# jkomijani/normflow_

Measured on AMD Instinct MI355X. Metric: lattice configs/sec (forward+logdet), higher is better.
Workload: dtype f32; 1 GPU; 32x32x32x32 phi^4 lattice, 8 RQ-spline coupling layers (knots_len 16, ConvAct 1-8-8-46, k=3, tanh), batch 1024 per GPU, forward + log|det J|, no_grad; global_batch=1024, parallelism=dp1

## Files before the change

include/normflow_hip.h:

```cpp
#ifndef NORMFLOW_HIP_H
#define NORMFLOW_HIP_H

#include <stddef.h>
#include <stdint.h>

#ifdef __cplusplus
extern "C" {
#endif

#define NF_VERSION 301

enum nf_dtype { NF_F32 = 0, NF_F64 = 1, NF_F16 = 2, NF_F16_FIELD = 3 };
enum nf_layout { NF_LAYOUT_FULL = 0, NF_LAYOUT_PAIR = 1 };
enum nf_extrap { NF_EXTRAP_NONE = 0, NF_EXTRAP_LINEAR = 1, NF_EXTRAP_ANTI = 2 };
enum nf_status {
  NF_OK = 0,
  NF_EINVAL = -1,
  NF_EWORKSPACE = -2,
  NF_ELAUNCH = -3
};

typedef struct nf_rqs_opts {
  int32_t m;
  int32_t extrap_left;
// ... 106 lines not shown

enum nf_pade_kind { NF_TANH = 1, NF_PADE11 = 11, NF_PADE22 = 22, NF_PADE32 = 32 };
size_t nf_pade_workspace_bytes(int64_t B, int64_t outer, int64_t C, int64_t inner);
int nf_pade(const void *x, const void *d0, const void *d1, const void *log0, void *y, void *logj, int64_t B,
            int64_t outer, int64_t C, int64_t inner, int kind, int inverse, int per_site, void *workspace,
            size_t workspace_bytes, int dtype, void *stream);
int nf_pade_vjp(const void *x, const void *d0, const void *d1, const void *grad_y, const void *grad_logj,
                void *grad_x, double *grad_d, int64_t B, int64_t outer, int64_t C, int64_t inner, int kind,
                int inverse, int per_site, void *workspace, size_t workspace_bytes, int dtype, void *stream);

int nf_spectral_supported(const int32_t *lat, int ndim, int dtype, int for_vjp);
size_t nf_spectral_workspace_bytes(const int32_t *lat, int ndim, int64_t B, int dtype);
int nf_spectral_filter(const void *x, const void *w_half, const void *zero_new, void *y, void *zero_old,
                       const int32_t *lat, int ndim, int64_t B, int dtype, void *stream);
int nf_spectral_filter_vjp(const void *x, const void *g, const void *w_half, int zero_replaced, void *gx, void *gw_half,
                           void *gzero, void *workspace, size_t workspace_bytes, const int32_t *lat, int ndim, int64_t B,
                           int dtype, void *stream);

int nf_conv_two_site(int cout, int compact, int l3, int k3);
int nf_conv_cin_pad(int cin);
int nf_conv_ntiles(int cout);
int nf_conv_packed_steps(int cin, int ntaps);
enum { NF_OUT_SPLIT16 = 2 };
int nf_conv_fwd(const void *in, const void *wfrag, const void *bias, void *out, int64_t B,
                const int32_t *lattice, const int32_t *ksize, int cin, int cout, int act,
                int compact, int active_parity, int dtype, void *stream);
enum { NF_WLAYOUT_FRAGMENT = 0, NF_WLAYOUT_ROWPACK = 1, NF_WLAYOUT_SPLIT16 = 2 };
int nf_conv_weight_layout(const int32_t *lattice, const int32_t *ksize, int cin, int cout, int compact,
                          int fused, int dtype);
int nf_conv_split16_supported(const int32_t *lattice, const int32_t *ksize, int cin, int cout, int act);
int nf_conv_affine_split16(const void *in16, const void *wsplit, const void *bias, const void *x_active, const void *log0,
                           void *y, void *logj, int64_t B, const int32_t *lattice, int active_parity, int inverse,
                           int flags, void *workspace, size_t workspace_bytes, void *stream);
int nf_conv_first_split16_supported(const int32_t *lattice, const int32_t *ksize, int cout, int act);
int nf_conv_first_split16(const void *in, const void *wsplit, const void *bias, void *out16, int64_t B,
                          const int32_t *lattice, int act, void *stream);
int nf_conv_fwd_split16(const void *in16, const void *wsplit, const void *bias, void *out16, int64_t B,
                        const int32_t *lattice, int act, void *stream);
typedef struct nf_conv_layer_plan {
  int32_t path;
  int32_t weight_layout;
  int32_t mt;
  int32_t two_site;
  int32_t packed;
  int32_t box[4];
  int32_t nbox[4];
  int32_t plane_stride;
  int32_t channels_per_pass;
  int32_t launches;
  int64_t lds_bytes;
  int64_t partials;
} nf_conv_layer_plan;
int nf_conv_plan(const int32_t *lattice, const int32_t *ksize, int cin, int cout, int compact, int fused, int dtype,
                 int64_t B, nf_conv_layer_plan *out);
int nf_conv_last_path(void);

enum { NF_CONV_UNIT_INPUT = 1, NF_CONV_SPLIT16_INPUT = 2, NF_CONV_FIELD_F16 = 4 };
int nf_conv_rqs_supported(int cout, int m);
int nf_conv_rqs_split16_supported(const int32_t *lattice, int cout, int m);
int nf_conv_rqs(const void *in, const void *wfrag, const void *bias, const void *x_active,
                const void *log0, void *y, void *logj, int64_t B, const int32_t *lattice,
                const int32_t *ksize, int cin, int cout, int active_parity,
                const nf_rqs_opts *opts, int inverse, int flags, void *workspace, size_t workspace_bytes,
                int dtype, void *stream);

int nf_phi4_action(const void *cfgs, void *action, int64_t B, const int32_t *lattice, double w0, double w2,
// ... 325 lines not shown
```

normflow__amd/_hip.py:

```python
import ctypes as C
import math
import os
import threading
import weakref

import torch

_HERE = os.path.dirname(os.path.abspath(__file__))
LIB_PATH = os.path.join(_HERE, "lib", "libnormflow_hip.so")

NF_F32, NF_F64, NF_F16, NF_F16_FIELD = 0, 1, 2, 3
LAYOUT_FULL, LAYOUT_PAIR = 0, 1
EXTRAP = {None: 0, 'none': 0, 'linear': 1, 'anti': 2, 'anti-periodic': 2}


OPT_SPLIT16, OPT_PIPE = 0, 1


class NormflowHipError(RuntimeError):
    pass


class RqsOpts(C.Structure):
    _fields_ = [("m", C.c_int32), ("extrap_left", C.c_int32), ("extrap_right", C.c_int32),
# ... 828 lines not shown
    lo = (w2 - hi.float()).half()
    out = torch.empty(27, 2, 64, 8, dtype=torch.float16, device=w.device)
    for k, part in enumerate((hi, lo)):
        out[:, k] = part.permute(2, 3, 0, 1).reshape(27, 64, 8)
    return out.contiguous()


def pack_conv_weight_split16_stacked(w):
    assert tuple(w.shape) == (8, 8, 3, 3, 3, 3)
    wr = w.reshape(8, 8, 9, 3, 3).float() * SPLIT16_WEIGHT_SCALE
    hi = wr.half()
    lo = (wr - hi.float()).half()
    parts = torch.stack((hi, lo))[:, :, :, :8]
    v = parts.reshape(2, 8, 8, 2, 4, 3, 3).permute(3, 5, 6, 4, 0, 1, 2)
    stacked = v.reshape(18, 64, 8)
    return torch.cat((stacked, pack_conv_weight_split16_two_site(w).reshape(54, 64, 8))).contiguous()


def pack_conv_weight_split16_first(w):
    assert tuple(w.shape) == (8, 1, 3, 3, 3, 3)
    wr = w.reshape(8, 27, 3).float() * SPLIT16_WEIGHT_SCALE
    w2 = wr.new_zeros(16, 32, 4)
    w2[:8, :27, :3] = wr
    w2[8:, :27, 1:] = wr
    hi = w2.half()
    lo = (w2 - hi.float()).half()
    out = torch.empty(4, 2, 64, 8, dtype=torch.float16, device=w.device)
    for k, part in enumerate((hi, lo)):
        v = part.reshape(16, 4, 4, 2, 4).permute(1, 2, 0, 3, 4)
        out[:, k] = v.reshape(4, 64, 8)
    return out.contiguous()


def conv_first_split16(x, weight, bias, act, weight_src=None):
    lib = load()
    B = x.shape[0]
    lat4 = _lat4(x.shape[2:])
    V = _sites(x.shape[2:])
    wsp = _cached_pack(weight if weight_src is None else weight_src, 'first16', pack_conv_weight_split16_first)
    bias = None if bias is None else bias.detach().float().contiguous()
    out = torch.empty((B, V, 16), dtype=torch.float16, device=x.device)
    for b0, b1 in _slabs(B, max(1, min(MAX_B, ((1 << 31) - 1) // V))):
        _check(lib.nf_conv_first_split16(_ptr(x[b0:b1]), _ptr(wsp), _ptr(bias), _ptr(out[b0:b1]), b1 - b0, lat4,
                                         int(act), _stream()), "nf_conv_first_split16")
    return out


def _split16_site_index(L3, device):
    slot = torch.arange(L3 // 2, device=device)
    return torch.stack((2 * slot, (2 * slot - 1) % L3))


def to_split16(h):
    B, Cc = h.shape[:2]
    L3 = h.shape[-1]
    if Cc != 8 or L3 % 2:
        raise NormflowHipError("to_split16: 8 channels and an even fastest axis expected")
    hp = h.reshape(B, 8, -1, L3).float()
    idx = _split16_site_index(L3, h.device)
    g = hp[..., idx].permute(0, 2, 3, 4, 1)
    hi = g.half()
    lo = (g - hi.float()).half()
    return torch.stack((hi, lo), dim=2).reshape(B, -1, 16).contiguous()


def from_split16(h16, lattice):
    B = h16.shape[0]
    L3 = lattice[-1]
    t = h16.reshape(B, -1, 2, 2, L3 // 2, 8).float()
    v = t[:, :, 0] + t[:, :, 1]
    idx = _split16_site_index(L3, h16.device)
    out = torch.empty((B, v.shape[1], L3, 8), dtype=torch.float32, device=h16.device)
# ... 96 lines not shown
        packed = build(probe)
        idx = (packed.reshape(-1).round().to(torch.int64) - 1).to(torch.int32).contiguous()
        ent = (idx, tuple(packed.shape))
        _GATHER_MAPS[key] = ent
    return ent


def _pack_by_gather(weight, gather_map):
    idx, shape = gather_map
    w = weight.contiguous()
    out = torch.empty(shape, dtype=w.dtype, device=w.device)
    _check(load().nf_gather_pad(_ptr(w), _ptr(idx), _ptr(out), idx.numel(), w.numel(), w.element_size(), _stream()), "nf_gather_pad")
    return out


def _conv_weight_map(shape, device, lat4, k4, cin, cout, compact, two_site, transposed, dtype_code):
    layout = load().nf_conv_weight_layout(lat4, k4, cin, cout, int(compact), 0, dtype_code)
    ksize = list(shape[2:])

    def build(w):
        if transposed:
            w = w.flip(list(range(2, w.dim()))).transpose(0, 1)
        if two_site:
            w2 = w.new_zeros((16, cin) + tuple(ksize[:-1]) + (ksize[-1] + 1,))
            w2[:cout, ..., :ksize[-1]] = w
            w2[8:8 + cout, ..., 1:] = w
            w = w2
        return conv_weight_for_layer(w, lat4, k4, cin, cout, compact, False, dtype_code)

    return _gather_map(shape, device, build, (transposed, two_site, tuple(lat4), tuple(k4), cin, cout, int(compact), dtype_code,
                                              layout))


def _conv_launch(x, weight, bias, act, compact, parity, weight_src=None, transposed=False):
    lib = load()
    B, cin = x.shape[:2]
    lat = list(x.shape[2:])
    cout, ksize = weight.shape[1 if transposed else 0], list(weight.shape[2:])
    d = len(lat)
    lat4, k4 = _lat4(lat, ksize)
    split16 = compact == 2
    if (split16 and cin == 1 and cout == 8 and d == 4 and x.dtype == torch.float32
            and _weights_fit_fp16(weight if weight_src is None else weight_src)
            and lib.nf_conv_first_split16_supported(lat4, k4, cout, act)):
        return conv_first_split16(x, weight, bias, act, weight_src)
    if split16 and not (lib.nf_conv_two_site(cout, 0, lat[-1], ksize[-1]) and cout == 8 and x.dtype == torch.float32):
        raise NormflowHipError("split-fp16 output needs an fp32 two-site layer with 8 output channels")
    two_site = bool(lib.nf_conv_two_site(cout, 0 if split16 else int(compact), lat[-1], ksize[-1]))
    eff_compact = False if (two_site and split16) else compact
    wfrag = _pack_by_gather(weight, _conv_weight_map(weight.shape, weight.device, lat4, k4, cin, cout, eff_compact, two_site,
                                                     transposed, _dtype_code(x)))
    V = _sites(lat)
    if split16:
        out = torch.empty((B, V, 16), dtype=torch.float16, device=x.device)
    else:
        out = torch.empty((B, cout, V // 2) if compact else (B, cout) + tuple(lat), dtype=x.dtype, device=x.device)
    for b0, b1 in _slabs(B):
        _check(lib.nf_conv_fwd(_ptr(x[b0:b1]), _ptr(wfrag), _ptr(bias), _ptr(out[b0:b1]), b1 - b0, lat4, k4,
                               cin, cout, act, int(compact), int(parity), _dtype_code(x), _stream()), "nf_conv_fwd")
    return out


def _compact_to_full(t, lattice, parity):
    _require_device(t)
    B, Cc, Vh = t.shape
    t = t.contiguous()
    full = torch.empty((B, Cc) + tuple(lattice), dtype=t.dtype, device=t.device)
    _check(load().nf_expand_pairs(_ptr(t), _ptr(full), B * Cc, _lat4(lattice), int(parity), _dtype_code(t), _stream()),
           "nf_expand_pairs")
    return full


def absmax_bits(t):
    bits = torch.empty(1, dtype=torch.int32, device=t.device)
    _check(load().nf_absmax_bits(_ptr(t), t.numel(), _ptr(bits), _stream()), "nf_absmax_bits")
    return bits


# ... 273 lines not shown
        lattice = tuple(h.shape[2:])
        lat4 = _lat4(lattice)
        cout = weight.shape[0]
        bits = absmax_bits(h)
        src, is16 = FusedLastRqsFn._source(h, bits, lat4)
        wsp = pack_conv_weight_split16(weight.detach().float())
        b = None if bias is None else bias.detach().float().contiguous()
        gz = torch.empty((B, cout, V // 2), dtype=torch.float32, device=h.device)
        gx = torch.empty_like(xpt)
        gy, glogj = gy.contiguous(), glogj.contiguous()
        work = torch.empty(4, dtype=torch.float32, device=h.device)
        _check(lib.nf_cotangent_pow2(_ptr(gy), gy.numel(), _ptr(glogj), glogj.numel(), _ptr(work), _stream()), "nf_cotangent_pow2")
        gys, gls = torch._foreach_mul([gy, glogj], work[2])
        _check(lib.nf_conv_rqs_split16_vjp(_ptr(src), is16, _ptr(wsp), _ptr(b), cout, _ptr(xpt), _ptr(gys),
                                           _ptr(gls), _ptr(gz), _ptr(gx), B, lat4, int(ctx.parity), _ptr(bits),
                                           C.byref(ctx.opts), int(bool(ctx.inverse)), _stream()), "nf_conv_rqs_split16_vjp")
        gh = gw = gb = None
        gbits = absmax_bits(gz)
        if ctx.needs_input_grad[0]:
            wt = weight.detach().flip([2, 3, 4, 5]).transpose(0, 1).contiguous()
            gh = conv_input_grad_split16(gz, wt, gbits, ctx.parity, lattice, weight)
        if ctx.needs_input_grad[1] or (bias is not None and ctx.needs_input_grad[2]):
            got = conv_weight_grad(h, gz, weight.shape[2:], gbits, ctx.parity)
            if got is not None:
                gw, gb = got
        if (ctx.needs_input_grad[0] and gh is None) or ((ctx.needs_input_grad[1] or ctx.needs_input_grad[2]) and gw is None):
            raise NormflowHipError("FusedLastRqsFn.backward: the split-fp16 gradient kernels refused a layer the forward pass took")
        if bias is None:
            gb = None
        torch._foreach_mul_([t for t in (gh, gw, gb, gx) if t is not None], work[3])
        return gh, gw, gb, gx, (glogj if ctx.has_log0 else None), None, None, None


def conv_layer(x, weight, bias, act=0, compact=False, parity=0):
    if torch.is_grad_enabled() and (x.requires_grad or weight.requires_grad or (bias is not None and bias.requires_grad)):
        if act == 5:
            return torch.abs(ConvFn.apply(x, weight, bias, 0, compact, parity))
        return ConvFn.apply(x, weight, bias, act, compact, parity)
    x = x.contiguous()
    return _conv_launch(x, weight.detach(), None if bias is None else bias.detach(), act, compact, parity, weight_src=weight)


def conv_affine_split16(h16, weight, bias, x_active, log0, parity, inverse, lattice, out=None):
    _require_device(h16, weight, bias, x_active, log0)
    lib = load()
    B, V = x_active.shape
    x_active = x_active.contiguous()
    lat4 = _lat4(lattice)
    def pack_affine(w):
        w8 = w.new_zeros((8, 8, 3, 3, 3, 3), dtype=torch.float32)
        w8[:2] = w.float()
        return pack_conv_weight_split16_stacked(w8)
    wsp = _cached_pack(weight, 'affine16s', pack_affine)
    b8 = torch.zeros(8, dtype=torch.float32, device=x_active.device)
    if bias is not None:
        b8[:2] = bias.detach().float()
    field16 = x_active.dtype == torch.float16
    if out is None:
        y = torch.empty_like(x_active)
        logj = torch.empty(B, dtype=torch.float32, device=x_active.device)
    else:
        y, logj = out
    ws = _workspace(min(B, MAX_B), V, x_active.device)
    for b0, b1 in _slabs(B):
        _check(lib.nf_conv_affine_split16(_ptr(h16[b0:b1]), _ptr(wsp), _ptr(b8), _ptr(x_active[b0:b1]), _ptr(_slab(log0, b0, b1)),
                                          _ptr(y[b0:b1]), _ptr(logj[b0:b1]), b1 - b0, lat4, int(parity), int(inverse),
                                          4 if field16 else 0, _ptr(ws), ws.numel(), _stream()), "nf_conv_affine_split16")
    return y, logj


def conv_rqs(h, weight, bias, x_active, log0, parity, opts, inverse, unit_input=False, lattice=None, out=None):
    _require_device(h, weight, bias, x_active, log0)
    lib = load()
# ... 1174 lines not shown
```

normflow__amd/csrc/nf_conv_c.hip:

```cpp
#include <hip/hip_runtime.h>
#include <hip/hip_fp16.h>
#include "nf_conv_core.h"

namespace nf {

typedef _Float16 f16x8 __attribute__((ext_vector_type(8)));
typedef _Float16 f16x4 __attribute__((ext_vector_type(4)));

namespace c2 {
constexpr int SEG = 32;
#ifndef NF_C2_IROW
#define NF_C2_IROW 80
#endif
constexpr int IROW = NF_C2_IROW;
constexpr int MAXROWS = 36;
constexpr int PLANE = 2 * MAXROWS * IROW;
constexpr int NPL = 4;
constexpr int LDS_BYTES = NPL * PLANE;
constexpr float kInvWScale = 1.0f / 1024.0f;
}

__device__ __forceinline__ float act_affine_c(float a, float c1, float c0, float al, float ga) {
  const float t = __builtin_amdgcn_exp2f(__builtin_fmaf(a, c1, c0));
  return __builtin_fmaf(al, __builtin_amdgcn_rcpf(1.0f + t), ga);
// ... 204 lines not shown
      stage_advance();
      stage_live = sci < ncols_my;
      if (stage_live) stage_issue(spl);
    }
    if (compute) {
#pragma unroll
      for (int t = 0; t < (HK ? 1 : 2); ++t) {
        if (tz[t] < NT) {
          f16x4 hi, lo;
#pragma unroll
          for (int r = 0; r < 4; ++r) {
            const float a = am[t][r] + ac[t][r];
            const float v = act_affine_c(a, kc1, kc0[r], kal, kga);
            const _Float16 h0 = static_cast<_Float16>(v);
            hi[r] = h0;
            lo[r] = static_cast<_Float16>(v - static_cast<float>(h0));
          }
          if (lane_ok) {
            unsigned char *d = (HK ? ((p & 8) ? ocol[1] : ocol[0]) : ocol[t]) + unsigned(z) * unsigned(RB) + lane_o;
            *reinterpret_cast<f16x4 *>(d) = hi;
            *reinterpret_cast<f16x4 *>(d + HB) = lo;
          }
        }
      }
    }
    lds_barrier();
    if (++pl > L2) {
      pl = -1;
      if (++cci < ncols_my) open_column(cci);
    }
  }
}

}

using namespace nf;

extern "C" int nf_conv_first_split16_supported(const int32_t *lattice, const int32_t *ksize, int cout, int act) {
  if (!nf::option(NF_OPT_SPLIT16) || !lattice || !ksize || cout != 8) return 0;
  if (act != kActTanh && act != kActSigmoid) return 0;
  for (int mu = 0; mu < 4; ++mu)
    if (ksize[mu] != 3) return 0;
  return split16_lattice_ok(lattice) ? 1 : 0;
}

extern "C" int nf_conv_first_split16(const void *in, const void *wsplit, const void *bias, void *out16, int64_t B,
                                     const int32_t *lattice, int act, void *stream_) {
  hipStream_t stream = static_cast<hipStream_t>(stream_);
  NF_REQUIRE(in && wsplit && out16 && lattice, "nf_conv_first_split16: NULL pointer");
  const int32_t k3[4] = {3, 3, 3, 3};
  NF_REQUIRE(nf_conv_first_split16_supported(lattice, k3, 8, act), "nf_conv_first_split16: layer not supported (needs a fastest axis of 32 + 16 n sites, even other extents, tanh / sigmoid)");
  NF_REQUIRE(B >= 0 && B <= 65535, "nf_conv_first_split16: batch outside [0, 65535]");
  if (B == 0) return NF_OK;
  ConvArgs A{};
  A.in = in; A.wfrag = wsplit; A.bias = bias; A.out = out16;
  set_lattice_k3(A, lattice);
  A.cin = 1; A.cout = 8; A.act = act;
  A.box[0] = lattice[0] % 4 == 0 ? 4 : 2;
  A.box[1] = lattice[1] % 4 == 0 ? 4 : 2;
  A.nitems = B * int64_t(lattice[0] / A.box[0]) * int64_t(lattice[1] / A.box[1]) * int64_t((lattice[3] / 2 + 15) / 16);
  NF_REQUIRE(B * A.V < (int64_t(1) << 31), "nf_conv_first_split16: batch x volume >= 2^31 sites, split the batch");
  NF_REQUIRE(cu_count() > 0, "nf_conv_first_split16: no device properties");
  const int nseg = (lattice[3] / 2 + 15) / 16;
  const int64_t per_seg = A.nitems / nseg;
  auto go = [&](bool hk) {
    const int64_t grid = persistent_grid(2, A.nitems, false);
    if (hk)
      hipLaunchKernelGGL(conv_c2_kernel<true>, dim3(unsigned(grid)), dim3(512), c2::LDS_BYTES, stream, A);
    else
      hipLaunchKernelGGL(conv_c2_kernel<false>, dim3(unsigned(grid)), dim3(512), c2::LDS_BYTES, stream, A);
  };
  if (((lattice[3] / 2) & 15) == 8 && A.box[0] == 4 && A.box[1] == 4) {
    if (nseg > 1) {
      A.seg_lo = 0; A.seg_n = nseg - 1; A.nitems = per_seg * (nseg - 1);
      go(false);
    }
    A.seg_lo = nseg - 1; A.seg_n = 1; A.nitems = per_seg;
    go(true);
  } else {
    A.seg_lo = 0; A.seg_n = nseg;
    go(false);
  }
  return check_launch("conv split-fp16 first-layer kernel");
}
```

normflow__amd/nn/scalar/cntr_couplings_.py:

```python
import torch

from .couplings_ import Coupling_
from .couplings_ import ShiftCoupling_, AffineCoupling_
from .couplings_ import RQSplineCoupling_, MultiRQSplineCoupling_


class _Absent:

    def __set_name__(self, owner, name):
        self._name = name

    def __get__(self, obj, cls=None):
        raise AttributeError(f"{(cls or type(obj)).__name__} has no {self._name}: a controlled block takes (x, control)")


class DirectCntrCoupling_(Coupling_):

    parts_forward = _Absent()
    parts_backward = _Absent()

    def _as_control(self, control, like):
        control = control.detach()
        if control.device != like.device or control.dtype != like.dtype:
            control = control.to(device=like.device, dtype=like.dtype)
        return control

    def _cntr_parts(self, inverse, parts, control, log0):
        atom = self.atomic_backward if inverse else self.atomic_forward
        ctl = self._as_control(control, parts[0])
        order = reversed(range(len(self.nets))) if inverse else range(len(self.nets))
        for k in order:
            p = k % 2
            parts[p], log0 = atom(x_active=parts[p], x_frozen=ctl if k == 0 else parts[1 - p], parity=p,
                                  net=self.nets[k], log0=log0)
        return parts, log0

    def forward(self, x_and_control, log0=0):
        x, control = x_and_control
        parts, log0 = self._cntr_parts(False, list(self.mask.split(x)), control, log0)
        return (self.mask.cat(*parts), control), log0

    def backward(self, x_and_control, log0=0):
        x, control = x_and_control
        parts, log0 = self._cntr_parts(True, list(self.mask.split(x)), control, log0)
        return (self.mask.cat(*parts), control), log0


class CntrCoupling_(DirectCntrCoupling_):

    def __init__(self, *args, control_generator=None, **kwargs):
        super().__init__(*args, **kwargs)
        self.control_generator = control_generator
# ... 47 lines not shown
```

normflow__amd/nn/scalar/couplings_.py:

```python
from abc import ABC, abstractmethod

import torch

from .._core import Module_
from ... import _hip
from ...lib.spline import RQSpline

PARAM_SLAB_BYTES = 6 << 30
HIDDEN_SLAB_BYTES = 32 << 30
HIDDEN_SLAB_FLOOR = 8 << 30
_DEVICE_TOTAL = {}


TRAIN_FUSED_MIN_LOGIT_BYTES = 1 << 30


def set_training_fusion(min_logit_bytes):
    global TRAIN_FUSED_MIN_LOGIT_BYTES
    old = TRAIN_FUSED_MIN_LOGIT_BYTES
    TRAIN_FUSED_MIN_LOGIT_BYTES = int(min_logit_bytes)
    return old


def set_slab_bytes(params=None, hidden=None):
# ... 22 lines not shown

def _fixed_knots(knots, like):
    if knots is None:
        return None
    k = torch.as_tensor(knots)
    if k.dim() != 1:
        raise NotImplementedError("only 1-D fixed knots_x / knots_y are supported")
    return k.detach().to(device=like.device, dtype=like.dtype).contiguous()


def _knots_len(n_channels, kx, ky):
    n_fixed = (kx is not None) + (ky is not None)
    m, rest = divmod(n_channels + 2 - n_fixed, 3 - n_fixed)
    return (None if rest else m), n_fixed


class Coupling_(Module_, ABC):

    def __init__(self, nets, *, mask, channels_axis=1, label='coupling_'):
        super().__init__(label=label)
        self.nets = torch.nn.ModuleList(nets)
        self.mask = mask
        self.channels_axis = channels_axis
        self._act_cache = {}

    def forward(self, x, log0=0):
        parts, log0 = self.parts_forward(list(self.mask.split(x)), log0)
        return self.mask.cat(*parts), log0

    def backward(self, x, log0=0):
        parts, log0 = self.parts_backward(list(self.mask.split(x)), log0)
        return self.mask.cat(*parts), log0

    def parts_forward(self, parts, log0=0):
        for k, net in enumerate(self.nets):
            p = k % 2
            parts[p], log0 = self.atomic_forward(x_active=parts[p], x_frozen=parts[1 - p],
                                                 parity=p, net=net, log0=log0)
        return parts, log0

    def parts_backward(self, parts, log0=0):
        for k in reversed(range(len(self.nets))):
            p = k % 2
            parts[p], log0 = self.atomic_backward(x_active=parts[p], x_frozen=parts[1 - p],
                                                  parity=p, net=self.nets[k], log0=log0)
        return parts, log0

    @abstractmethod
    def atomic_forward(self, *, x_active, x_frozen, parity, net, log0=0):
        pass

    @abstractmethod
    def atomic_backward(self, *, x_active, x_frozen, parity, net, log0=0):
        pass

    def preprocess_fz(self, x):
        return x.unsqueeze(self.channels_axis)

    def preprocess(self, x):
        return x.unsqueeze(self.channels_axis)

    def postprocess(self, x):
        return x.squeeze(self.channels_axis)

    def _ctor_kwargs(self):
        return dict(label=self.label, channels_axis=self.channels_axis)

    def transfer(self, scale_factor=1, mask=None, **extra):
        nets = [net.transfer(scale_factor=scale_factor) for net in self.nets]
        return self.__class__(nets, mask=self.mask if mask is None else mask, **self._ctor_kwargs())

    def _activity(self, parity, lattice_shape, device):
        key = (parity, tuple(lattice_shape), str(device))
        hit = self._act_cache.get(key)
        if hit is None:
            hit = _activity_bytes(self.mask, parity, lattice_shape, device)
            self._act_cache = {key: hit, **{k: v for k, v in self._act_cache.items() if k[0] != parity}}
        return hit

    def _pair_parity(self, parity):
        if not getattr(self.mask, 'pairable', False) or not hasattr(self.mask, 'checkerboard_parity'):
            return None
        return self.mask.checkerboard_parity(parity)

    def _check_density(self):
        if self.propagate_density:
            raise NotImplementedError("propagate_density=True (per-site densities) is not provided by "
                                      "this coupling's kernels, which reduce log|J| per sample")

    def _no_grad_only(self, x_active, x_frozen, net):
        if _needs_grad(x_active, x_frozen, net):
            raise NotImplementedError("propagate_density=True is an inference path here (per-site densities have no VJP "
                                      "kernel); wrap the call in torch.no_grad()")

    def _density_slabs(self, x_active, x_frozen, net, n_out_hint, one_slab):
        B = x_active.shape[0]
        n_out = getattr(net, 'conv_kwargs', {}).get('out_channels', n_out_hint)
        per_sample = n_out * x_active[0].numel() * x_active.element_size()
        val, sites = torch.empty_like(x_active), torch.empty_like(x_active)
        for b0, b1 in self._slabs(B, per_sample):
            val[b0:b1], sites[b0:b1] = one_slab(x_active[b0:b1], x_frozen[b0:b1])
        return val, sites

    def _affine_density_atom(self, inverse, x_active, x_frozen, parity, net, log0):
        self._no_grad_only(x_active, x_frozen, net)
        act = self._activity(parity, x_active.shape[1:], x_active.device)

        def one_slab(xa, xf):
            params, layout = self._params(net, xf, None)
            val, _, sites = _hip.affine_sites(xa.reshape(xa.shape[0], -1), params, act, None, layout, inverse)
            return val.reshape(xa.shape), sites.reshape(xa.shape)
        val, sites = self._density_slabs(x_active, x_frozen, net, 2, one_slab)
        return val, log0 + sites

    def _params(self, net, x_frozen, parity=None):
        if x_frozen.dtype == torch.float16:
# ... 71 lines not shown
        if self.propagate_density:
            val, _ = self._run_atom(k, x_active, x_frozen, parity, net, 0, 1, density_ok=True)
            return val, log0
        val, lj = self._run_atom(k, x_active, x_frozen, parity, net, log0, 1)
        return val, (lj if torch.is_tensor(log0) or log0 != 0 else log0)

    def atomic_forward(self, **kw):
        return self._atom(False, **kw)

    def atomic_backward(self, **kw):
        return self._atom(True, **kw)


class AffineCoupling_(Coupling_):

    def _fused_atom(self, inverse, x_active, x_frozen, parity, net, log0):
        if _needs_grad(x_active, x_frozen, net):
            return None
        if (self.propagate_density or self.channels_axis != 1 or not hasattr(net, 'hidden_and_last')
                or x_active.dtype not in (torch.float32, torch.float16) or x_active.dim() != 5):
            return None
        a = self._pair_parity(parity)
        if a is None or net.conv_kwargs['out_channels'] != 2:
            return None
        B = x_active.shape[0]
        v = x_active.reshape(B, -1).contiguous()
        l0 = _hip._log0_tensor(log0, v, B)
        hidden = max(net.conv_kwargs['hidden_sizes'] or [1])
        val = torch.empty_like(v)
        lj = torch.empty(B, dtype=torch.float32, device=v.device)
        lattice = tuple(x_frozen.shape[1:])
        for b0, b1 in self._hidden_slabs(v, hidden):
            xf = x_frozen[b0:b1]
            got = net.hidden_and_last(self.preprocess_fz(xf.float() if xf.dtype == torch.float16 else xf), last_kind='affine')
            if got is None:
                return None
            h16, last, unit, split = got
            _hip.conv_affine_split16(h16, last.weight, last.bias, v[b0:b1], None if l0 is None else l0[b0:b1], a, inverse,
                                     lattice, out=(val[b0:b1], lj[b0:b1]))
        return val.reshape(x_active.shape), lj

    def _atom(self, inverse, *, x_active, x_frozen, parity, net, log0=0):
        if self.propagate_density:
            return self._affine_density_atom(inverse, x_active, x_frozen, parity, net, log0)
        fused = self._fused_atom(inverse, x_active, x_frozen, parity, net, log0)
        if fused is None and getattr(net, 'conv_kwargs', {}).get('out_channels') == 2:
            fused = self._small_lattice_atom(1, inverse, x_active, x_frozen, parity, net, log0)
        if fused is not None:
            return fused
        k = lambda v, p, l0, act, layout: _hip.AffineCouplingFn.apply(v, p, l0, act, layout, inverse)
        return self._run_atom(k, x_active, x_frozen, parity, net, log0, 2)

    def atomic_forward(self, **kw):
        return self._atom(False, **kw)

    def atomic_backward(self, **kw):
        return self._atom(True, **kw)


class RQSplineCoupling_(Coupling_):

    def __init__(self, nets, *, mask, xlim=(0, 1), ylim=(0, 1), knots_x=None, knots_y=None,
                 extrap={}, **kwargs):
        super().__init__(nets, mask=mask, **kwargs)
        self.xlim, self.xwidth = xlim, xlim[1] - xlim[0]
        self.ylim, self.ywidth = ylim, ylim[1] - ylim[0]
        self.knots_x = knots_x
# ... 14 lines not shown
        if _needs_grad(x_active, x_frozen, net):
            return None
        if (self.propagate_density or self.channels_axis != 1 or self.knots_x is not None
                or self.knots_y is not None or not hasattr(net, 'hidden_and_last')
                or x_active.dtype not in (torch.float32, torch.float16)):
            return None
        a = self._pair_parity(parity)
        n_out = net.conv_kwargs['out_channels']
        if a is None or (n_out + 2) % 3:
            return None
        opts = _hip.make_rqs_opts((n_out + 2) // 3, self.xlim, self.ylim, self.extrap, _hip.LAYOUT_PAIR)
        small = self._small_lattice_atom(0, inverse, x_active, x_frozen, parity, net, log0, opts)
        if small is not None:
            return small
        if (hasattr(net, '_wide_plan') and x_active.dtype == torch.float32 and x_active.dim() == 5
                and net._wide_plan(self.preprocess_fz(x_frozen[:1])) is not None):
            return None
        any_kernel = bool(_hip.load().nf_conv_rqs_supported(n_out, (n_out + 2) // 3))
        if not any_kernel and not hasattr(net, '_fuse_plan'):
            return None
        B = x_active.shape[0]
        v = x_active.reshape(B, -1)
        l0 = _hip._log0_tensor(log0, v, B)
        hidden = max(net.conv_kwargs['hidden_sizes'] or [1])
        v = v.contiguous()
        val = torch.empty_like(v)
        lj = torch.empty(B, dtype=torch.float32 if v.dtype == torch.float16 else v.dtype, device=v.device)
        for b0, b1 in self._hidden_slabs(v, hidden):
            xf = x_frozen[b0:b1]
            xin = self.preprocess_fz(xf.float() if xf.dtype == torch.float16 else xf)
            planned = net._fuse_plan(xin) if hasattr(net, '_fuse_plan') else None
            if planned is not None and not any_kernel and not planned[4]:
                return None
            got = net.hidden_and_last(xin, planned=planned) if planned is not None else net.hidden_and_last(xin)
            if got is None:
                return None
            h, last, unit, split = got
            _hip.conv_rqs(h, last.weight, last.bias, v[b0:b1], None if l0 is None else l0[b0:b1], a,
                          opts, inverse, unit_input=unit, lattice=tuple(x_frozen.shape[1:]) if split else None,
                          out=(val[b0:b1], lj[b0:b1]))
        return val.reshape(x_active.shape), lj

    def make_spline(self, out):
        return RQSpline(out, xlim=self.xlim, ylim=self.ylim, knots_x=self.knots_x, knots_y=self.knots_y,
                        extrap=self.extrap, knots_axis=self.channels_axis)

    def _hack(self, *, x_active, x_frozen, parity, net):
        with torch.no_grad():
            out = net(self.preprocess_fz(x_frozen))
            spline = self.make_spline(out)
            act = self._activity(parity, x_active.shape[1:], x_active.device)
            fx, logg = spline._map(x_active, False, True, True, activity=act, log=True)
        return spline, fx, logg

    def _density_atom(self, inverse, x_active, x_frozen, parity, net, log0):
        self._no_grad_only(x_active, x_frozen, net)
        act = self._activity(parity, x_active.shape[1:], x_active.device)

        def one_slab(xa, xf):
            spline = self.make_spline(net(self.preprocess_fz(xf)))
            return spline._map(xa, inverse, True, True, activity=act, log=True)
        val, logg = self._density_slabs(x_active, x_frozen, net, 46, one_slab)
        return val, log0 + logg

    def _train_fused_atom(self, inverse, x_active, x_frozen, parity, net, log0):
        if not _needs_grad(x_active, x_frozen, net):
            return None
# ... 117 lines not shown
```

normflow__amd/nn/scalar/modules.py:

```python
import copy
import math

import torch

from .convNd import Conv4d
from ... import _hip

LN2 = math.log(2.0)


class Abs(torch.nn.Module):
    def forward(self, x):
        return torch.abs(x)


class AvgNeighborPool(torch.nn.Module):

    def forward(self, x):
        dims = range(1, x.ndim)
        return sum(torch.roll(x, s, d) for d in dims for s in (1, -1)) / (2 * len(dims))


ACTIVATIONS = torch.nn.ModuleDict({
    'tanh': torch.nn.Tanh(), 'relu': torch.nn.ReLU(), 'leaky_relu': torch.nn.LeakyReLU(),
# ... 126 lines not shown
        plan = self._plan()
        if plan is None or plan[-1][1] != 0:
            return None
        wbs = [self._wb(conv) for conv, _ in plan]
        got = self._fuse_plan_for(x, plan, wbs, last_kind)
        hidden = [w.shape[0] for w, _ in wbs[:-1]]
        if ((got is None or not got[4]) and len(plan) > 2 and x.dim() == 6 and hidden and all(h == hidden[0] for h in hidden)
                and 1 <= hidden[0] < 8 and all(w.dim() == 6 and tuple(w.shape[2:]) == (3, 3, 3, 3) for w, _ in wbs)
                and wbs[0][0].shape[1] == 1 and wbs[0][0].dtype == torch.float32):
            n = len(plan)
            wb8 = [self._pad8(plan[i][0], w, b, pad_out=i < n - 1, pad_in=i > 0) for i, (w, b) in enumerate(wbs)]
            got8 = self._fuse_plan_for(x, plan, wb8, last_kind)
            if got8 is not None and got8[4]:
                return got8
        return got

    def _fuse_plan_for(self, x, plan, wbs, last_kind):
        import types
        plan = [(types.SimpleNamespace(weight=w, bias=b), act) for (w, b), (_, act) in zip(wbs, plan)]
        if plan[0][0].weight.dtype == torch.float32 and x.dtype == torch.float16:
            x = x.float()
        if not _hip.conv_supported(x, plan[0][0].weight):
            return None
        unit = len(plan) > 1 and plan[-2][1] in (_hip.ACT_CODES['tanh'], _hip.ACT_CODES['expit'])
        if last_kind == 'affine':
            lw = plan[-1][0].weight
            split = (unit and len(plan) > 2 and x.dtype == torch.float32 and lw.dim() == 6 and tuple(lw.shape) == (2, 8, 3, 3, 3, 3)
                     and _hip._weights_fit_fp16(lw))
        else:
            split = unit and len(plan) > 2 and self._wants_split16(x, plan)
        chain = split and self._split16_chain(x, plan)
        return plan, x, unit, split, chain

    def hidden_and_last(self, x, last_kind='rqs', planned=None):
        got = planned if planned is not None else self._fuse_plan(x, last_kind)
        if got is None:
            return None
        plan, x, unit, split, chain = got
        if last_kind == 'affine' and not chain:
            return None
        lat = tuple(x.shape[2:])
        for n, (conv, act) in enumerate(plan[:-1]):
            last_hidden = n == len(plan) - 2
            if chain and n > 0:
                x = _hip.conv_layer_split16(x, conv.weight, conv.bias, act, lat)
            else:
                x = _hip.conv_layer(x, conv.weight, conv.bias, act,
                                    compact=2 if ((chain and n == 0) or (split and last_hidden)) else False)
        return x, plan[-1][0], unit, split

    def small3d_plan(self):
        cd = self.conv_kwargs['conv_dim']
        if self.conv_kwargs.get('pre_act') is not None or cd not in (2, 3):
            return None
        plan = self._plan()
        ok_act = (_hip.ACT_CODES['tanh'], _hip.ACT_CODES['expit'])
        if plan is None or len(plan) != 3 or plan[0][1] not in ok_act or plan[1][1] not in ok_act or plan[2][1] != 0:
            return None
        wbs = [self._wb(conv) for conv, _ in plan]
        (w1, b1), (w2, b2), (w3, b3) = wbs
        h = w1.shape[0]
        if (w1.dtype != torch.float32 or not w1.is_cuda or any(tuple(w.shape[2:]) != (3,) * cd for w, _ in wbs) or w1.shape[1] != 1
                or not 1 <= h <= 8 or tuple(w2.shape[:2]) != (h, h) or w3.shape[1] != h or w3.shape[0] > 46):
            return None
        if not all(_hip._weights_fit_fp16(w) for w, _ in wbs):
            return None
        ver = _param_key(*wbs)
        hit = self.__dict__.get('_small3d')
        if hit is None or hit[0] != ver:
            with torch.no_grad():
                def pad(w, no, ni):
                    w = w.detach().float()
                    if cd == 2:
                        w3 = w.new_zeros(tuple(w.shape[:2]) + (3, 3, 3))
                        w3[:, :, 1] = w
                        w = w3
                    return torch.nn.functional.pad(w, (0, 0, 0, 0, 0, 0, 0, ni - w.shape[1], 0, no - w.shape[0]))
                padb = lambda b, no: None if b is None else torch.nn.functional.pad(b.detach().float(), (0, no - b.shape[0]))
                packed = _hip.pack_small3d_weights(pad(w1, 8, 1), pad(w2, 8, 8), pad(w3, w3.shape[0], 8))
                biases = (padb(b1, 8), padb(b2, 8), padb(b3, w3.shape[0]))
            hit = (ver, packed, biases, (plan[0][1], plan[1][1]), int(w3.shape[0]))
# ... 198 lines not shown
```

Measured before the change: 983.4 configs/s.

## Add frozen-parity first-layer split16 conv kernel skipping masked-zero input taps

Adds a specialized first-layer (1->8 channel) split-fp16 conv kernel used when the frozen input is checkerboard-masked, so half the sites are known zero. Weights are repacked per parity so each MFMA only covers the nonzero taps. Input is staged through a multi-plane LDS ring with overlapped global loads, and the parity is threaded from the coupling layers down to the launch. This aims to roughly halve the MMA and load work of the first conv. It adds a new persistent kernel and a second weight blob, and correctness depends on the input really being zero on the frozen parity.

After: 998.1 configs/s, median of 6. 1.02x the previous value.

```diff
diff --git a/include/normflow_hip.h b/include/normflow_hip.h
--- a/include/normflow_hip.h
+++ b/include/normflow_hip.h
@@ -162,6 +162,10 @@
 int nf_conv_affine_split16(const void *in16, const void *wsplit, const void *bias, const void *x_active, const void *log0,
                            void *y, void *logj, int64_t B, const int32_t *lattice, int active_parity, int inverse,
                            int flags, void *workspace, size_t workspace_bytes, void *stream);
+#define NF_FIRST_FROZEN_EVEN 0x100
+#define NF_FIRST_FROZEN_ODD 0x200
+#define NF_FIRST_FRAGS_MAX 0xff
+#define NF_FIRST_FRAGS(n) ((int)(n) << 16)
 int nf_conv_first_split16_supported(const int32_t *lattice, const int32_t *ksize, int cout, int act);
 int nf_conv_first_split16(const void *in, const void *wsplit, const void *bias, void *out16, int64_t B,
                           const int32_t *lattice, int act, void *stream);
diff --git a/normflow__amd/_hip.py b/normflow__amd/_hip.py
--- a/normflow__amd/_hip.py
+++ b/normflow__amd/_hip.py
@@ -884,12 +884,52 @@
     return out.contiguous()
 
 
-def conv_first_split16(x, weight, bias, act, weight_src=None):
+def _first_parity_taps():
+    j3 = torch.full((2, 2, 32, 2), 3, dtype=torch.long, device='cpu')
+    for sigma in range(2):
+        for r in range(27):
+            e = sigma ^ ((r // 9 + (r // 3) % 3 + r % 3 + 1) & 1)
+            for shift in range(2):
+                for tp in range(2):
+                    j = 1 - e + 2 * tp - shift
+                    if 0 <= j <= 2:
+                        j3[sigma, shift, r, tp] = j
+    return j3
+
+
+_FIRST_PARITY_TAPS = []
+FIRST_FROZEN_FLAG = (0x100, 0x200)
+FIRST_PARITY_FRAGS = 16 << 16
+
+
+def pack_conv_weight_split16_first_parity(w):
+    assert tuple(w.shape) == (8, 1, 3, 3, 3, 3)
+    if not _FIRST_PARITY_TAPS:
+        _FIRST_PARITY_TAPS.append(_first_parity_taps())
+    j3 = _FIRST_PARITY_TAPS[0].to(w.device)
+    wr = w.new_zeros(8, 32, 4, dtype=torch.float32)
+    wr[:, :27, :3] = w.reshape(8, 27, 3).float() * SPLIT16_WEIGHT_SCALE
+    rows = torch.arange(32, device=w.device).view(1, 1, 32, 1).expand_as(j3)
+    w2 = wr[:, rows, j3].permute(1, 2, 0, 3, 4).reshape(2, 16, 32, 2)
+    hi = w2.half()
+    lo = (w2 - hi.float()).half()
+    out = torch.empty(2, 2, 2, 64, 8, dtype=torch.float16, device=w.device)
+    for k, part in enumerate((hi, lo)):
+        v = part.reshape(2, 16, 2, 4, 4, 2).permute(0, 2, 3, 1, 4, 5)
+        out[:, :, k] = v.reshape(2, 2, 64, 8)
+    return torch.cat((pack_conv_weight_split16_first(w).reshape(8, 64, 8), out.reshape(8, 64, 8))).contiguous()
+
+
+def conv_first_split16(x, weight, bias, act, weight_src=None, frozen_parity=None):
     lib = load()
     B = x.shape[0]
     lat4 = _lat4(x.shape[2:])
     V = _sites(x.shape[2:])
-    wsp = _cached_pack(weight if weight_src is None else weight_src, 'first16', pack_conv_weight_split16_first)
+    if frozen_parity is None:
+        wsp = _cached_pack(weight if weight_src is None else weight_src, 'first16', pack_conv_weight_split16_first)
+    else:
+        wsp = _cached_pack(weight if weight_src is None else weight_src, 'first16p', pack_conv_weight_split16_first_parity)
+        act = int(act) | FIRST_FROZEN_FLAG[int(frozen_parity) & 1] | FIRST_PARITY_FRAGS
     bias = None if bias is None else bias.detach().float().contiguous()
     out = torch.empty((B, V, 16), dtype=torch.float16, device=x.device)
     for b0, b1 in _slabs(B, max(1, min(MAX_B, ((1 << 31) - 1) // V))):
@@ -1052,7 +1092,7 @@
                                               layout))
 
 
-def _conv_launch(x, weight, bias, act, compact, parity, weight_src=None, transposed=False):
+def _conv_launch(x, weight, bias, act, compact, parity, weight_src=None, transposed=False, frozen_parity=None):
     lib = load()
     B, cin = x.shape[:2]
     lat = list(x.shape[2:])
@@ -1063,7 +1103,7 @@
     if (split16 and cin == 1 and cout == 8 and d == 4 and x.dtype == torch.float32
             and _weights_fit_fp16(weight if weight_src is None else weight_src)
             and lib.nf_conv_first_split16_supported(lat4, k4, cout, act)):
-        return conv_first_split16(x, weight, bias, act, weight_src)
+        return conv_first_split16(x, weight, bias, act, weight_src, frozen_parity)
     if split16 and not (lib.nf_conv_two_site(cout, 0, lat[-1], ksize[-1]) and cout == 8 and x.dtype == torch.float32):
         raise NormflowHipError("split-fp16 output needs an fp32 two-site layer with 8 output channels")
     two_site = bool(lib.nf_conv_two_site(cout, 0 if split16 else int(compact), lat[-1], ksize[-1]))
@@ -1403,13 +1443,14 @@
         return gh, gw, gb, gx, (glogj if ctx.has_log0 else None), None, None, None
 
 
-def conv_layer(x, weight, bias, act=0, compact=False, parity=0):
+def conv_layer(x, weight, bias, act=0, compact=False, parity=0, frozen_parity=None):
     if torch.is_grad_enabled() and (x.requires_grad or weight.requires_grad or (bias is not None and bias.requires_grad)):
         if act == 5:
             return torch.abs(ConvFn.apply(x, weight, bias, 0, compact, parity))
         return ConvFn.apply(x, weight, bias, act, compact, parity)
     x = x.contiguous()
-    return _conv_launch(x, weight.detach(), None if bias is None else bias.detach(), act, compact, parity, weight_src=weight)
+    return _conv_launch(x, weight.detach(), None if bias is None else bias.detach(), act, compact, parity, weight_src=weight,
+                        frozen_parity=frozen_parity if compact == 2 else None)
 
 
 def conv_affine_split16(h16, weight, bias, x_active, log0, parity, inverse, lattice, out=None):
diff --git a/normflow__amd/csrc/nf_conv_c.hip b/normflow__amd/csrc/nf_conv_c.hip
--- a/normflow__amd/csrc/nf_conv_c.hip
+++ b/normflow__amd/csrc/nf_conv_c.hip
@@ -260,12 +260,251 @@
   }
 }
 
+namespace c3 {
+constexpr int ROWB = 160;
+constexpr int H1 = 6, NROWS = 36;
+constexpr int Z0B = H1 * ROWB + 32;
+constexpr int PLANE = H1 * Z0B + 160;
+constexpr int NPL = 4;
+constexpr int LDS_BYTES = (NPL + 2) * PLANE;
+constexpr int T1OFF = 2 * Z0B;
+constexpr int NFRAG_DENSE = 8, NFRAG = 16;
+static_assert((ROWB / 4) % 64 == 40 && (Z0B / 4) % 64 == 56 && (PLANE / 4) % 64 == 56, "the conflict-free pitches");
+}
+
+template <int V>
+struct IntC { static constexpr int value = V; };
+
+__global__ __launch_bounds__(512, 2) void conv_c3_kernel(ConvArgs A) {
+  using namespace c3;
+  extern __shared__ __align__(16) unsigned char smem_c3[];
+  const int lane = threadIdx.x & 63;
+  const int wave = __builtin_amdgcn_readfirstlane(threadIdx.x >> 6);
+  const int g = lane >> 4, p = lane & 15;
+  const int n0 = A.L[0] >> 2, n1 = A.L[1] >> 2, ncol = n0 * n1;
+  const int L2 = A.L[2], L3 = A.L[3];
+  const int RB = L3 * 32, HB = L3 * 16;
+  const int seg_n = L3 >> 5;
+  const int phi = A.parity;
+  const int total = int(A.nitems);
+  const int nwg = gridDim.x;
+  if (int(blockIdx.x) >= total) return;
+  const int ncols_my = (total - int(blockIdx.x) + nwg - 1) / nwg;
+  auto decode = [&](int ci, int &b, int &i0, int &i1, int &hs) {
+    int gc = int(blockIdx.x) + ci * nwg;
+    hs = gc % seg_n;
+    gc /= seg_n;
+    b = gc / ncol;
+    const int c = gc - b * ncol;
+    i0 = c / n1;
+    i1 = c - i0 * n1;
+  };
+
+  const int wz0 = wave >> 2, wz1 = wave & 3;
+  const int sigma0 = (wz0 + wz1 + phi) & 1;
+  f16x8 wh[2][2], wl[2][2];
+  {
+    const f16x8 *__restrict__ wsp = static_cast<const f16x8 *>(A.wfrag) + NFRAG_DENSE * 64 + lane;
+#pragma unroll
+    for (int sp = 0; sp < 2; ++sp)
+#pragma unroll
+      for (int sl = 0; sl < 2; ++sl) {
+        const int f = ((sigma0 ^ sp) * 2 + sl) * 2;
+        wh[sp][sl] = wsp[f * 64];
+        wl[sp][sl] = wsp[(f + 1) * 64];
+      }
+  }
+  float bv4[4], kc0[4];
+#pragma unroll
+  for (int r = 0; r < 4; ++r) bv4[r] = A.bias ? static_cast<const float *>(A.bias)[4 * (g & 1) + r] : 0.f;
+  const bool is_tanh = A.act != kActSigmoid;
+  const float kcs = is_tanh ? 2.885390081777927f : -1.4426950408889634f;
+  const float kal = is_tanh ? -2.0f : 1.0f, kga = is_tanh ? 1.0f : 0.0f;
+#pragma unroll
+  for (int r = 0; r < 4; ++r) kc0[r] = kcs * bv4[r];
+  const float kc1 = kcs * c2::kInvWScale;
+
+  typedef unsigned u32x2 __attribute__((ext_vector_type(2)));
+  typedef __attribute__((address_space(3))) const u32x2 lds_win_t;
+  unsigned wadr[2][4];
+#pragma unroll
+  for (int sl = 0; sl < 2; ++sl)
+#pragma unroll
+    for (int h = 0; h < 4; ++h) {
+      int r = 16 * sl + 4 * g + h;
+      r = r < 27 ? r : (r == 27 ? 26 : (r - 4 < 26 ? r - 4 : 26));
+      const int j0 = r / 9, j1 = (r / 3) % 3, j2 = r % 3;
+      wadr[sl][h] = unsigned(size_t((__attribute__((address_space(3))) unsigned char *)smem_c3)) +
+                    unsigned(j2 * PLANE + (wz0 + j0) * Z0B + (wz1 + j1) * ROWB + 8 * p);
+    }
+
+  const float *__restrict__ inb = static_cast<const float *>(A.in);
+  const bool second = wave == 0;
+  unsigned soff[2][2][2];
+  float sv[2][2] = {{0.f, 0.f}, {0.f, 0.f}};
+  auto open_stage_column = [&](int ci, const float *&base) {
+    int b, i0, i1, hs;
+    decode(ci, b, i0, i1, hs);
+    base = inb + int64_t(b) * A.V;
+#pragma unroll
+    for (int q = 0; q < 2; ++q) {
+      const int wid = q * 512 + int(threadIdx.x);
+      const int row = wid >> 4, pw = wid & 15;
+      const int hz0 = row / H1, hz1 = row - hz0 * H1;
+      int x0 = 4 * i0 + hz0 - 1, x1 = 4 * i1 + hz1 - 1;
+      x0 = x0 < 0 ? x0 + A.L[0] : (x0 >= A.L[0] ? x0 - A.L[0] : x0);
+      x1 = x1 < 0 ? x1 + A.L[1] : (x1 >= A.L[1] ? x1 - A.L[1] : x1);
+      const int rowbase = (x0 * A.L[1] + x1) * (L2 * L3);
+#pragma unroll
+      for (int pp = 0; pp < 2; ++pp) {
+        const int e = (phi + hz0 + hz1 + pp) & 1;
+        int s0 = c2::SEG * hs + 2 * pw - e, s1 = s0 + 2;
+        s0 = s0 < 0 ? s0 + L3 : s0;
+        s1 = s1 >= L3 ? s1 - L3 : s1;
+        soff[q][pp][0] = unsigned(rowbase + s0) * 4u;
+        soff[q][pp][1] = unsigned(rowbase + s1) * 4u;
+      }
+    }
+  };
+  unsigned sdst[2];
+#pragma unroll
+  for (int q = 0; q < 2; ++q) {
+    const int wid = q * 512 + int(threadIdx.x), row = wid >> 4;
+    sdst[q] = unsigned((row / H1) * Z0B + (row % H1) * ROWB + (wid & 15) * 8);
+  }
+  auto stage_issue = [&](const float *base, int x2, int pp) {
+    const int z = x2 < 0 ? x2 + L2 : (x2 >= L2 ? x2 - L2 : x2);
+    const unsigned char *pb = reinterpret_cast<const unsigned char *>(base + z * L3);
+    sv[0][0] = *reinterpret_cast<const float *>(pb + soff[0][pp][0]);
+    sv[0][1] = *reinterpret_cast<const float *>(pb + soff[0][pp][1]);
+    if (second) {
+      sv[1][0] = *reinterpret_cast<const float *>(pb + soff[1][pp][0]);
+      sv[1][1] = *reinterpret_cast<const float *>(pb + soff[1][pp][1]);
+    }
+  };
+  auto stage_commit = [&](int slot) {
+    unsigned char *ph = smem_c3 + slot * PLANE;
+#pragma unroll
+    for (int q = 0; q < 2; ++q) {
+      if (q == 0 || second) {
+        f16x4 w;
+        w[0] = static_cast<_Float16>(sv[q][0]);
+        w[1] = static_cast<_Float16>(sv[q][1]);
+        w[2] = static_cast<_Float16>(sv[q][0] - static_cast<float>(w[0]));
+        w[3] = static_cast<_Float16>(sv[q][1] - static_cast<float>(w[1]));
+        *reinterpret_cast<f16x4 *>(ph + sdst[q]) = w;
+        if (slot < 2) *reinterpret_cast<f16x4 *>(ph + NPL * PLANE + sdst[q]) = w;
+      }
+    }
+  };
+
+  unsigned char *__restrict__ outb = static_cast<unsigned char *>(A.out);
+  const int64_t sampleB = A.V * 32;
+  unsigned char *orow[2] = {nullptr, nullptr};
+  unsigned lane_o = 0;
+  auto open_column = [&](int ci) {
+    int b, i0, i1, hs;
+    decode(ci, b, i0, i1, hs);
+    lane_o = unsigned(pair_row_offset(2 * (16 * hs + p) + (g >> 1), L3) + (g & 1) * 8);
+#pragma unroll
+    for (int t = 0; t < 2; ++t)
+      orow[t] = outb + int64_t(b) * sampleB + int64_t(((4 * i0 + wz0 + 2 * t) * A.L[1] + 4 * i1 + wz1) * L2) * RB;
+  };
+
+  const int EPC = L2 + 2;
+  const int nent = ncols_my * EPC;
+  int sci = 0, spl = -1;
+  const float *sbase = nullptr;
+  auto stage_advance = [&]() {
+    if (++spl > L2) {
+      spl = -1;
+      if (++sci < ncols_my) open_stage_column(sci, sbase);
+    }
+  };
+  open_stage_column(0, sbase);
+  stage_issue(sbase, spl, 1); stage_commit(0); stage_advance();
+  stage_issue(sbase, spl, 0); stage_commit(1); stage_advance();
+  stage_issue(sbase, spl, 1); stage_commit(2); stage_advance();
+  bool stage_live = sci < ncols_my;
+  if (stage_live) stage_issue(sbase, spl, 0);
+  lds_barrier();
+
+  int cci = 0, pl = -1;
+  open_column(0);
+  auto step = [&](auto kc) {
+    constexpr int k = decltype(kc)::value;
+    const bool compute = pl <= L2 - 2;
+    f32x4 am[2], ac[2];
+    if (compute) {
+      am[0] = am[1] = ac[0] = ac[1] = f32x4{0.f, 0.f, 0.f, 0.f};
+      __builtin_amdgcn_s_setprio(2);
+#pragma unroll
+      for (int sl = 0; sl < 2; ++sl) {
+        union { f16x8 v; unsigned w[4]; } fh[2], fl[2];
+#pragma unroll
+        for (int h = 0; h < 4; ++h)
+#pragma unroll
+          for (int t = 0; t < 2; ++t) {
+            const u32x2 win = *(lds_win_t *)(wadr[sl][h] + unsigned(k * PLANE + t * T1OFF));
+            fh[t].w[h] = win.x;
+            fl[t].w[h] = win.y;
+          }
+#pragma unroll
+        for (int t = 0; t < 2; ++t) {
+          am[t] = __builtin_amdgcn_mfma_f32_16x16x32_f16(wh[k & 1][sl], fh[t].v, am[t], 0, 0, 0);
+          ac[t] = __builtin_amdgcn_mfma_f32_16x16x32_f16(wl[k & 1][sl], fh[t].v, ac[t], 0, 0, 0);
+          ac[t] = __builtin_amdgcn_mfma_f32_16x16x32_f16(wh[k & 1][sl], fl[t].v, ac[t], 0, 0, 0);
+        }
+      }
+      __builtin_amdgcn_s_setprio(0);
+    }
+    if (stage_live) {
+      stage_commit((k + 3) & (NPL - 1));
+      stage_advance();
+      stage_live = sci < ncols_my;
+      if (stage_live) stage_issue(sbase, spl, (k + 1) & 1);
+    }
+    if (compute) {
+#pragma unroll
+      for (int t = 0; t < 2; ++t) {
+        f16x4 hi, lo;
+#pragma unroll
+        for (int r = 0; r < 4; ++r) {
+          const float a = am[t][r] + ac[t][r];
+          const float v = act_affine_c(a, kc1, kc0[r], kal, kga);
+          const _Float16 h0 = static_cast<_Float16>(v);
+          hi[r] = h0;
+          lo[r] = static_cast<_Float16>(v - static_cast<float>(h0));
+        }
+        unsigned char *d = orow[t] + lane_o;
+        *reinterpret_cast<f16x4 *>(d) = hi;
+        *reinterpret_cast<f16x4 *>(d + HB) = lo;
+        orow[t] += RB;
+      }
+    }
+    lds_barrier();
+    if (++pl > L2) {
+      pl = -1;
+      if (++cci < ncols_my) open_column(cci);
+    }
+  };
+  for (int e = 0; e < nent; e += 4) {
+    step(IntC<0>{});
+    step(IntC<1>{});
+    if (e + 2 >= nent) break;
+    step(IntC<2>{});
+    step(IntC<3>{});
+  }
+}
+
 }
 
 using namespace nf;
 
 extern "C" int nf_conv_first_split16_supported(const int32_t *lattice, const int32_t *ksize, int cout, int act) {
   if (!nf::option(NF_OPT_SPLIT16) || !lattice || !ksize || cout != 8) return 0;
+  if ((act & NF_FIRST_FROZEN_EVEN) && (act & NF_FIRST_FROZEN_ODD)) return 0;
+  act &= ~(NF_FIRST_FROZEN_EVEN | NF_FIRST_FROZEN_ODD | NF_FIRST_FRAGS(NF_FIRST_FRAGS_MAX));
   if (act != kActTanh && act != kActSigmoid) return 0;
   for (int mu = 0; mu < 4; ++mu)
     if (ksize[mu] != 3) return 0;
@@ -279,7 +518,27 @@
   const int32_t k3[4] = {3, 3, 3, 3};
   NF_REQUIRE(nf_conv_first_split16_supported(lattice, k3, 8, act), "nf_conv_first_split16: layer not supported (needs a fastest axis of 32 + 16 n sites, even other extents, tanh / sigmoid)");
   NF_REQUIRE(B >= 0 && B <= 65535, "nf_conv_first_split16: batch outside [0, 65535]");
+  const bool frozen = (act & (NF_FIRST_FROZEN_EVEN | NF_FIRST_FROZEN_ODD)) != 0;
+  const int phi = (act & NF_FIRST_FROZEN_ODD) ? 1 : 0;
+  const int nfrag = (act >> 16) & NF_FIRST_FRAGS_MAX;
+  act &= 0xff;
+  NF_REQUIRE(!frozen || nfrag >= c3::NFRAG,
+             "nf_conv_first_split16: a frozen-parity flag needs the weight blob with the parity fragments (NF_FIRST_FRAGS(16))");
   if (B == 0) return NF_OK;
+  if (frozen && lattice[3] % 32 == 0 && lattice[0] % 4 == 0 && lattice[1] % 4 == 0) {
+    ConvArgs A{};
+    A.in = in; A.wfrag = wsplit; A.bias = bias; A.out = out16;
+    set_lattice_k3(A, lattice);
+    A.cin = 1; A.cout = 8; A.act = act; A.parity = phi;
+    A.box[0] = A.box[1] = 4;
+    A.nitems = B * int64_t(lattice[0] / 4) * int64_t(lattice[1] / 4) * int64_t(lattice[3] / 32);
+    NF_REQUIRE(B * A.V < (int64_t(1) << 31), "nf_conv_first_split16: batch x volume >= 2^31 sites, split the batch");
+    NF_REQUIRE(A.V < (int64_t(1) << 29), "nf_conv_first_split16: volume >= 2^29 sites");
+    NF_REQUIRE(cu_count() > 0, "nf_conv_first_split16: no device properties");
+    const int64_t grid = persistent_grid(2, A.nitems, false);
+    hipLaunchKernelGGL(conv_c3_kernel, dim3(unsigned(grid)), dim3(512), c3::LDS_BYTES, stream, A);
+    return check_launch("conv split-fp16 first-layer kernel (frozen parity)");
+  }
   ConvArgs A{};
   A.in = in; A.wfrag = wsplit; A.bias = bias; A.out = out16;
   set_lattice_k3(A, lattice);
diff --git a/normflow__amd/nn/scalar/cntr_couplings_.py b/normflow__amd/nn/scalar/cntr_couplings_.py
--- a/normflow__amd/nn/scalar/cntr_couplings_.py
+++ b/normflow__amd/nn/scalar/cntr_couplings_.py
@@ -18,6 +18,7 @@
 
     parts_forward = _Absent()
     parts_backward = _Absent()
+    frozen_input_is_masked = False
 
     def _as_control(self, control, like):
         control = control.detach()
diff --git a/normflow__amd/nn/scalar/couplings_.py b/normflow__amd/nn/scalar/couplings_.py
--- a/normflow__amd/nn/scalar/couplings_.py
+++ b/normflow__amd/nn/scalar/couplings_.py
@@ -78,6 +78,8 @@
         parts, log0 = self.parts_backward(list(self.mask.split(x)), log0)
         return self.mask.cat(*parts), log0
 
+    frozen_input_is_masked = True
+
     def parts_forward(self, parts, log0=0):
         for k, net in enumerate(self.nets):
             p = k % 2
@@ -128,6 +130,12 @@
         if not getattr(self.mask, 'pairable', False) or not hasattr(self.mask, 'checkerboard_parity'):
             return None
         return self.mask.checkerboard_parity(parity)
+
+    def _frozen_parity(self, parity):
+        a = self._pair_parity(parity)
+        if not self.frozen_input_is_masked or a is None or type(self).preprocess_fz is not Coupling_.preprocess_fz:
+            return None
+        return 1 - int(a)
 
     def _check_density(self):
         if self.propagate_density:
@@ -265,7 +273,8 @@
         lattice = tuple(x_frozen.shape[1:])
         for b0, b1 in self._hidden_slabs(v, hidden):
             xf = x_frozen[b0:b1]
-            got = net.hidden_and_last(self.preprocess_fz(xf.float() if xf.dtype == torch.float16 else xf), last_kind='affine')
+            got = net.hidden_and_last(self.preprocess_fz(xf.float() if xf.dtype == torch.float16 else xf), last_kind='affine',
+                                      frozen_parity=self._frozen_parity(parity))
             if got is None:
                 return None
             h16, last, unit, split = got
@@ -346,7 +355,9 @@
             planned = net._fuse_plan(xin) if hasattr(net, '_fuse_plan') else None
             if planned is not None and not any_kernel and not planned[4]:
                 return None
-            got = net.hidden_and_last(xin, planned=planned) if planned is not None else net.hidden_and_last(xin)
+            fzp = self._frozen_parity(parity)
+            got = (net.hidden_and_last(xin, planned=planned, frozen_parity=fzp) if planned is not None
+                   else net.hidden_and_last(xin, frozen_parity=fzp))
             if got is None:
                 return None
             h, last, unit, split = got
diff --git a/normflow__amd/nn/scalar/modules.py b/normflow__amd/nn/scalar/modules.py
--- a/normflow__amd/nn/scalar/modules.py
+++ b/normflow__amd/nn/scalar/modules.py
@@ -182,7 +182,7 @@
         chain = split and self._split16_chain(x, plan)
         return plan, x, unit, split, chain
 
-    def hidden_and_last(self, x, last_kind='rqs', planned=None):
+    def hidden_and_last(self, x, last_kind='rqs', planned=None, frozen_parity=None):
         got = planned if planned is not None else self._fuse_plan(x, last_kind)
         if got is None:
             return None
@@ -196,7 +196,8 @@
                 x = _hip.conv_layer_split16(x, conv.weight, conv.bias, act, lat)
             else:
                 x = _hip.conv_layer(x, conv.weight, conv.bias, act,
-                                    compact=2 if ((chain and n == 0) or (split and last_hidden)) else False)
+                                    compact=2 if ((chain and n == 0) or (split and last_hidden)) else False,
+                                    frozen_parity=frozen_parity if (chain and n == 0) else None)
         return x, plan[-1][0], unit, split
 
     def small3d_plan(self):
```
